# bioinfo-pf-curie/mpiBWA

Hardware: AMD Instinct MI355X
Metric: Mreads/s (whole node) 2x150 bp PE vs GRCh38-size reference; SAM bit-match (higher is better)
Workload: dtype int32

## Files before the change

mpibwa_amd/csrc/chain_kernel.hip:

```cpp
#include <hip/hip_runtime.h>
#include <hipcub/hipcub.hpp>
#include <cstdlib>
#include <mutex>
#include <utility>
#include <vector>
#include "hip_util.h"
#include "device.h"
#include "sortutil.h"

namespace mbw {

namespace {

typedef long long i64;

#define CK_MAXCH 9
#define CK_MAXCH_SMALL 4
#define CK_MAXSEEDS_SMALL 16
#define CK_MAXSEEDS 64
#define CK_MAXSEEDS_BIG 255
enum { F_POS_LO = 0, F_POS_HI, F_FIRST_Q, F_LAST_R_LO, F_LAST_R_HI, F_LAST_Q, F_LAST_LEN, F_RID, F_N, F_W, F_KEPT, F_FIRSTOV, F_NFIELDS };

template <int MAXCH>
struct StoreLds {
	uint32_t *tab;
	uint8_t *cid_;
	uint8_t *ord_;
	uint8_t *tmp_;
	int lane;
	__device__ __forceinline__ uint32_t &f(int field, int id) const { return tab[(field * MAXCH + id) * 64 + lane]; }
	__device__ __forceinline__ uint8_t &cid(int k) const { return cid_[k * 64 + lane]; }
	__device__ __forceinline__ uint8_t &ord(int k) const { return ord_[k * 64 + lane]; }
	__device__ __forceinline__ uint8_t &tmp(int k) const { return tmp_[k * 64 + lane]; }
};

template <int MAXCH> __device__ __forceinline__ i64 st_pos(const StoreLds<MAXCH> &L, int id) { return (i64)((unsigned long long)L.f(F_POS_HI, id) << 32 | L.f(F_POS_LO, id)); }
template <int MAXCH> __device__ __forceinline__ i64 st_last_r(const StoreLds<MAXCH> &L, int id) { return (i64)((unsigned long long)L.f(F_LAST_R_HI, id) << 32 | L.f(F_LAST_R_LO, id)); }

template <int MAXCH>
struct MapArray {
	int n = 0;
	__device__ __forceinline__ int lower(const StoreLds<MAXCH> &L, i64 pos) const
	{
		int f = 0;
		while (f < n && st_pos(L, L.ord(f)) < pos) ++f;
		const int li = (f < n && st_pos(L, L.ord(f)) == pos) ? f : f - 1;
		return li >= 0 ? (int)L.ord(li) : -1;
	}
	__device__ __forceinline__ bool put(const StoreLds<MAXCH> &L, int id, i64 pos)
	{
		if (n == MAXCH) return false;
		int f = 0;
		while (f < n && st_pos(L, L.ord(f)) < pos) ++f;
		const int li = (f < n && st_pos(L, L.ord(f)) == pos) ? f : f - 1;
		for (int t = n; t > li + 1; --t) L.ord(t) = L.ord(t - 1);
		L.ord(li + 1) = (uint8_t)id;
		++n;
		return true;
	}
};

__device__ __forceinline__ int ck_pos2rid(const i64 *__restrict__ ann_off, int n_seqs, i64 l_pac, i64 pos_f)
{
	if (pos_f >= l_pac) return -1;
	int left = 0, mid = 0, right = n_seqs;
	while (left < right) {
		mid = (left + right) >> 1;
		if (pos_f >= ann_off[mid]) {
			if (mid == n_seqs - 1 || pos_f < ann_off[mid + 1]) break;
			left = mid + 1;
		} else right = mid;
	}
	return mid;
}
__device__ __forceinline__ i64 ck_depos(i64 l_pac, i64 pos) { return pos >= l_pac ? (l_pac << 1) - 1 - pos : pos; }

template <int MAXCH>
__device__ __forceinline__ int chain_read(const StoreLds<MAXCH> &L, const ChainParams &P, int rd, int ns, int lq, i64 so, const int *__restrict__ l_rep,
                                          const unsigned long long *__restrict__ sa, const int32_t *__restrict__ qbl, const i64 *__restrict__ ann_off,
                                          const uint8_t *__restrict__ ann_alt, int n_seqs, const int *__restrict__ gap, DevChain *__restrict__ chains,
                                          DevSeed *__restrict__ seeds, unsigned int *__restrict__ srt)
{
	const i64 l_pac = P.l_pac;
	auto S_R = [&](int k) -> i64 { return (i64)sa[so + k]; };
	auto S_Q = [&](int k) -> int { return qbl[2 * (so + k)]; };
	auto S_L = [&](int k) -> int { return qbl[2 * (so + k) + 1]; };
	auto members = [&](int id, auto fn) {
		for (int k = 0; k < ns; ++k)
			if (L.cid(k) == id) fn(k);
	};

	MapArray<MAXCH> map;
	int n_ch = 0;
	i64 c_lo = 0, c_hi = -1;
	int c_rid = -1;
	for (int k = 0; k < ns; ++k) {
		const i64 rb = S_R(k);
		const int qb = S_Q(k), len = S_L(k);
		L.cid(k) = 255;
		int rid;
		if (rb >= c_lo && rb + len <= c_hi && len > 0) rid = c_rid;
		else {
			if (rb < l_pac && rb + len > l_pac) rid = -2;
			else {
				const int rid_b = ck_pos2rid(ann_off, n_seqs, l_pac, ck_depos(l_pac, rb));
				const int rid_e = len > 0 ? ck_pos2rid(ann_off, n_seqs, l_pac, ck_depos(l_pac, rb + len - 1)) : rid_b;
				rid = rid_b == rid_e ? rid_b : -1;
			}
			if (rid >= 0) {
				const i64 o = ann_off[rid], l = ann_off[rid + 1] - o;
				if (rb < l_pac) { c_lo = o; c_hi = o + l; }
				else { c_lo = (l_pac << 1) - o - l; c_hi = (l_pac << 1) - o; }
				c_rid = rid;
			}
		}
		if (rid < 0) continue;
		const int id0 = map.lower(L, rb);
		bool merged = false;
		if (id0 >= 0) {
			const int id = id0;
			const i64 first_r = st_pos(L, id), last_r = st_last_r(L, id);
			const int first_q = (int)L.f(F_FIRST_Q, id), last_q = (int)L.f(F_LAST_Q, id), last_len = (int)L.f(F_LAST_LEN, id);
			const int qend = last_q + last_len;
			const i64 rend = last_r + last_len;
			if ((int)L.f(F_RID, id) == rid) {
				if (qb >= first_q && qb + len <= qend && rb >= first_r && rb + len <= rend) merged = true;
				else if (!((last_r < l_pac || first_r < l_pac) && rb >= l_pac)) {
					const i64 x = qb - last_q, y = rb - last_r;
					if (y >= 0 && x - y <= P.w && y - x <= P.w && x - last_len < P.max_chain_gap && y - last_len < P.max_chain_gap) {
						L.f(F_LAST_R_LO, id) = (uint32_t)rb; L.f(F_LAST_R_HI, id) = (uint32_t)((unsigned long long)rb >> 32);
						L.f(F_LAST_Q, id) = (uint32_t)qb; L.f(F_LAST_LEN, id) = (uint32_t)len;
						L.f(F_N, id) += 1;
						L.cid(k) = (uint8_t)id;
						merged = true;
					}
				}
			}
		}
		if (merged) continue;
		const int id = n_ch;
		if (id >= MAXCH) return -1;
		L.f(F_POS_LO, id) = (uint32_t)rb; L.f(F_POS_HI, id) = (uint32_t)((unsigned long long)rb >> 32);
		L.f(F_FIRST_Q, id) = (uint32_t)qb;
		L.f(F_LAST_R_LO, id) = (uint32_t)rb; L.f(F_LAST_R_HI, id) = (uint32_t)((unsigned long long)rb >> 32);
		L.f(F_LAST_Q, id) = (uint32_t)qb; L.f(F_LAST_LEN, id) = (uint32_t)len;
		L.f(F_RID, id) = (uint32_t)rid; L.f(F_N, id) = 1;
		if (!map.put(L, id, rb)) return -1;
		L.cid(k) = (uint8_t)id;
		++n_ch;
	}

	int n = 0;
	for (int t = 0; t < n_ch; ++t) {
		const int id = L.ord(t);
		i64 end = 0;
		int w = 0, wq;
		members(id, [&](int k) {
			const int qb = S_Q(k), len = S_L(k);
			if (qb >= end) w += len;
			else if (qb + len > end) w += (int)(qb + len - end);
			end = end > qb + len ? end : qb + len;
		});
		wq = w; w = 0; end = 0;
		members(id, [&](int k) {
			const i64 rb = S_R(k);
			const int len = S_L(k);
			if (rb >= end) w += len;
			else if (rb + len > end) w += (int)(rb + len - end);
			end = end > rb + len ? end : rb + len;
		});
		w = w < wq ? w : wq;
		w = w < 1 << 30 ? w : (1 << 30) - 1;
		const uint32_t w29 = (uint32_t)w & 0x1fffffffu;
		L.f(F_W, id) = w29; L.f(F_KEPT, id) = 0; L.f(F_FIRSTOV, id) = 0xffffffffu;
		if ((int)w29 < P.min_chain_weight) continue;
		L.ord(n++) = (uint8_t)id;
	}
	if (n == 0) return 0;
	static_assert(MAXCH <= 16, "ks_small_introsort_at is ks_introsort for at most 16 elements");
	ks_small_introsort_at(n, [&](int k) -> uint8_t & { return L.ord(k); },
	                      [&](int a_id, int b_id) -> bool { return (int)L.f(F_W, a_id) > (int)L.f(F_W, b_id); });
	auto BEG = [&](int t) -> int { return (int)L.f(F_FIRST_Q, L.ord(t)); };
	auto END = [&](int t) -> int { const int id = L.ord(t); return (int)L.f(F_LAST_Q, id) + (int)L.f(F_LAST_LEN, id); };
	auto ALT = [&](int t) -> int { return ann_alt[L.f(F_RID, L.ord(t))]; };
	int n_kept = 0;
	L.f(F_KEPT, L.ord(0)) = 3;
	L.tmp(n_kept++) = 0;
	for (int i = 1; i < n; ++i) {
		bool large_ovlp = false;
		int kk;
		for (kk = 0; kk < n_kept; ++kk) {
			const int j = L.tmp(kk);
			const int b_max = BEG(j) > BEG(i) ? BEG(j) : BEG(i);
			const int e_min = END(j) < END(i) ? END(j) : END(i);
			if (e_min > b_max && (!ALT(j) || ALT(i))) {
				const int li_ = END(i) - BEG(i), lj_ = END(j) - BEG(j);
				const int min_l = li_ < lj_ ? li_ : lj_;
				if ((float)(e_min - b_max) >= (float)min_l * P.mask_level && min_l < P.max_chain_gap) {
					large_ovlp = true;
					if (L.f(F_FIRSTOV, L.ord(j)) == 0xffffffffu) L.f(F_FIRSTOV, L.ord(j)) = (uint32_t)i;
					const int wi = (int)L.f(F_W, L.ord(i)), wj = (int)L.f(F_W, L.ord(j));
					if ((float)wi < (float)wj * P.drop_ratio && wj - wi >= P.min_seed_len << 1) break;
				}
			}
		}
		if (kk == n_kept) {
			L.tmp(n_kept++) = (uint8_t)i;
			L.f(F_KEPT, L.ord(i)) = large_ovlp ? 2 : 3;
		}
	}
	for (int kk = 0; kk < n_kept; ++kk) {
		const uint32_t fo = L.f(F_FIRSTOV, L.ord(L.tmp(kk)));
		if (fo != 0xffffffffu) L.f(F_KEPT, L.ord(fo)) = 1;
	}
	{
		int i = 0, cnt = 0;
		for (; i < n; ++i) {
			const uint32_t kp = L.f(F_KEPT, L.ord(i));
			if (kp == 0 || kp == 3) continue;
			if (++cnt >= P.max_chain_extend) break;
		}
		for (; i < n; ++i)
			if (L.f(F_KEPT, L.ord(i)) < 3) L.f(F_KEPT, L.ord(i)) = 0;
	}

	const float frac_rep = (float)l_rep[rd] / (float)lq;
	int n_out = 0;
	i64 cursor = so;
	for (int t = 0; t < n; ++t) {
		const int id = L.ord(t);
		if (L.f(F_KEPT, id) == 0) continue;
		int cs = 0;
		members(id, [&](int k) { L.tmp(cs++) = (uint8_t)k; });
		for (int a = 1; a < cs; ++a) {
			const uint8_t v = L.tmp(a);
			const int lv = S_L(v);
			int b = a;
			while (b > 0 && S_L(L.tmp(b - 1)) > lv) { L.tmp(b) = L.tmp(b - 1); --b; }
			L.tmp(b) = v;
		}
		const int rid = (int)L.f(F_RID, id);
		const i64 first_r = st_pos(L, id);
		i64 lo = l_pac << 1, hi = 0;
		for (int a = 0; a < cs; ++a) {
			const int k = L.tmp(a);
			DevSeed ds;
			ds.rbeg = S_R(k); ds.qbeg = S_Q(k); ds.len = S_L(k);
			seeds[cursor + a] = ds;
			srt[cursor + a] = (unsigned int)a;
			const i64 b = ds.rbeg - (ds.qbeg + gap[ds.qbeg]);
			const int tail = lq - ds.qbeg - ds.len;
			const i64 e = ds.rbeg + ds.len + (tail + gap[tail]);
			lo = b < lo ? b : lo;
			hi = e > hi ? e : hi;
		}
		DevChain d;
		i64 fb = ann_off[rid], fe = ann_off[rid + 1];
		if (first_r >= l_pac) { const i64 tt = fb; fb = (l_pac << 1) - fe; fe = (l_pac << 1) - tt; }
		d.far_beg = fb; d.far_end = fe;
		d.seed_beg = (int)cursor; d.n_seeds = cs; d.rid = rid; d.frac_rep = frac_rep;
		d.rmax0 = lo > 0 ? lo : 0;
		d.rmax1 = hi < l_pac << 1 ? hi : l_pac << 1;
		if (d.rmax0 < l_pac && l_pac < d.rmax1) {
			if (first_r < l_pac) d.rmax1 = l_pac;
			else d.rmax0 = l_pac;
		}
		d.rmax0 = d.rmax0 > fb ? d.rmax0 : fb;
		d.rmax1 = d.rmax1 < fe ? d.rmax1 : fe;
		chains[so + n_out] = d;
		++n_out;
		cursor += cs;
	}
	return n_out;
}

template <int MAXS, int MAXCH, int LO>
__global__ void __launch_bounds__(64)
chain_kernel(ChainParams P, int n_reads, const int *__restrict__ lens, const int *__restrict__ n_seeds, const int *__restrict__ l_rep,
             const i64 *__restrict__ seed_off, const unsigned long long *__restrict__ sa, const int32_t *__restrict__ qbl,
             const i64 *__restrict__ ann_off, const uint8_t *__restrict__ ann_alt, int n_seqs, const int *__restrict__ tab, int tab_stride,
             DevChain *__restrict__ chains, DevSeed *__restrict__ seeds, unsigned int *__restrict__ srt, int *__restrict__ n_chains,
             const int *__restrict__ list, const unsigned int *__restrict__ list_n)
{
	extern __shared__ uint32_t lds_raw[];
	StoreLds<MAXCH> L;
	L.lane = threadIdx.x;
	L.tab = lds_raw;
	L.cid_ = (uint8_t *)(lds_raw + F_NFIELDS * MAXCH * 64);
	L.ord_ = L.cid_ + (MAXS + 1) * 64;
	L.tmp_ = L.ord_ + 16 * 64;
	int rd = blockIdx.x * 64 + threadIdx.x;
	if (list) { if (rd >= (int)*list_n) return; rd = list[rd]; }
	if (rd >= n_reads) return;
	const int ns = n_seeds[rd], lq = lens[rd];
	const int *gap = tab, *noflt = tab + 5 * tab_stride;
	if (LO >= 0) { if (n_chains[rd] != -1 || ns <= LO) return; }
	else if (ns == 0) { n_chains[rd] = 0; return; }
	if (ns > MAXS || !noflt[lq]) { n_chains[rd] = -1; return; }
	n_chains[rd] = chain_read(L, P, rd, ns, lq, seed_off[rd], l_rep, sa, qbl, ann_off, ann_alt, n_seqs, gap, chains, seeds, srt);
}

__global__ void __launch_bounds__(256)
chain_pick_kernel(int n_reads, const int *__restrict__ lens, const int *__restrict__ n_seeds, const int *__restrict__ n_chains,
                  const int *__restrict__ noflt, int lo, int hi, int cap, int *__restrict__ list, unsigned int *__restrict__ count)
{
	const int rd = blockIdx.x * 256 + threadIdx.x;
	const bool mine = rd < n_reads && n_chains[rd] == -1 && n_seeds[rd] > lo && n_seeds[rd] <= hi && noflt[lens[rd]] != 0;
	const unsigned long long m = __ballot(mine);
	if (!m) return;
	const int lane = threadIdx.x & 63, lead = __ffsll((long long)m) - 1;
	unsigned int base = 0;
	if (lane == lead) base = atomicAdd(count, (unsigned int)__popcll(m));
	base = __shfl(base, lead);
	const unsigned int at = base + (unsigned int)__popcll(m & ((1ull << lane) - 1));
	if (mine && at < (unsigned int)cap) list[at] = rd;
}

#define HV_NONE 0xFFFFu
__host__ __device__ constexpr size_t hv_lds_bytes(int cap) { return (size_t)(cap + 64) * 24; }
__host__ __device__ constexpr size_t hv_scratch_bytes(int cap) { return (size_t)cap * (4 + 7 * 2 + 8 + 4) + 512; }
struct HvStore {
	uint32_t *rid;
	uint16_t *head, *cid, *next, *ord;
	uint32_t *last_off;
	uint16_t *first_q, *last_q, *last_len, *tail, *nmem;
};
__device__ __forceinline__ bool hv_lt(uint32_t a, uint32_t b) { return (a >> 16) > (b >> 16); }
#define HV_FRAMES 32
__device__ __forceinline__ void hv_sort(uint32_t *a, int n)
{
	int fs[HV_FRAMES], ft[HV_FRAMES], fd[HV_FRAMES];
	ks_introsort_at(n, [a](int k) -> uint32_t & { return a[k]; }, KsFramesAt{fs, ft, fd}, hv_lt);
}
__device__ __forceinline__ void hv_sync()
{
	__builtin_amdgcn_fence(__ATOMIC_RELEASE, "wavefront");
	__builtin_amdgcn_wave_barrier();
	__builtin_amdgcn_fence(__ATOMIC_ACQUIRE, "wavefront");
}
__device__ __forceinline__ int hv_bcast(int v) { return __builtin_amdgcn_readfirstlane(v); }

template <int CAP>
__global__ void __launch_bounds__(64)
chain_heavy_kernel(ChainParams P, const int *__restrict__ list, const unsigned int *__restrict__ list_n, unsigned int *work, int list_cap,
                   const int *__restrict__ lens, const int *__restrict__ n_seeds, const int *__restrict__ l_rep, const i64 *__restrict__ seed_off,
                   const unsigned long long *__restrict__ sa, const int32_t *__restrict__ qbl, const i64 *__restrict__ ann_off,
                   const uint8_t *__restrict__ ann_alt, int n_seqs, const int *__restrict__ gap, uint8_t *__restrict__ scratch,
                   DevChain *__restrict__ chains, DevSeed *__restrict__ seeds, unsigned int *__restrict__ srt, int *__restrict__ n_chains)
{
	extern __shared__ uint8_t hv_lds[];
	const int lane = threadIdx.x;
	i64 *spos = (i64 *)hv_lds;
	uint16_t *sid = (uint16_t *)(hv_lds + (size_t)(CAP + 64) * 22);
	uint32_t *skey = (uint32_t *)hv_lds;
	uint16_t *cbeg = (uint16_t *)(skey + CAP);
	uint16_t *cend = cbeg + CAP, *kidx = cend + CAP, *kfirst = kidx + CAP;
	uint8_t *calt = (uint8_t *)(kfirst + CAP), *ckept = calt + CAP;
	uint8_t *sb = scratch + (size_t)blockIdx.x * hv_scratch_bytes(CAP);
	HvStore S;
	S.rid = (uint32_t *)sb;
	S.head = (uint16_t *)(S.rid + CAP); S.cid = S.head + CAP; S.next = S.cid + CAP; S.ord = S.next + CAP;
	S.last_off = (uint32_t *)(hv_lds + (size_t)(CAP + 64) * 8);
	S.first_q = (uint16_t *)(S.last_off + CAP); S.last_q = S.first_q + CAP; S.last_len = S.last_q + CAP; S.tail = S.last_len + CAP; S.nmem = S.tail + CAP;
	uint16_t *g_first_q = S.ord + CAP, *g_end_q = g_first_q + CAP, *g_nmem = g_end_q + CAP;
	i64 *g_clo = (i64 *)(sb + (((size_t)CAP * 18 + 15) & ~(size_t)15));
	int *g_rid = (int *)(g_clo + CAP);
	const i64 l_pac = P.l_pac;
	const int n_list = (int)(*list_n < (unsigned int)list_cap ? *list_n : (unsigned int)list_cap);
	for (;;) {
		int t = 0;
		if (lane == 0) t = (int)atomicAdd(work, 1u);
		t = hv_bcast(t);
		if (t >= n_list) break;
		const int rd = hv_bcast(list[t]);
		const int ns = hv_bcast(n_seeds[rd]), lq = hv_bcast(lens[rd]);
		const i64 so = seed_off[rd];
		auto S_R = [&](int k) -> i64 { return (i64)sa[so + k]; };
		auto S_Q = [&](int k) -> int { return qbl[2 * (so + k)]; };
		auto S_L = [&](int k) -> int { return qbl[2 * (so + k) + 1]; };
		if (ns > CAP) continue;
		int n_ch = 0, ok = 1;
		{
			for (int k = lane; k < ns; k += 64) {
				const i64 rb = S_R(k);
				const int len = S_L(k);
				int rid;
				if (rb < l_pac && rb + len > l_pac) rid = -2;
				else {
					const int rid_b = ck_pos2rid(ann_off, n_seqs, l_pac, ck_depos(l_pac, rb));
					const int rid_e = len > 0 ? ck_pos2rid(ann_off, n_seqs, l_pac, ck_depos(l_pac, rb + len - 1)) : rid_b;
					rid = rid_b == rid_e ? rid_b : -1;
				}
				i64 lo = -1;
				if (rid >= 0) lo = rb < l_pac ? ann_off[rid] : (l_pac << 1) - ann_off[rid + 1];
				g_rid[k] = rid; g_clo[k] = lo;
			}
			hv_sync();
			i64 nx_rb = S_R(0), nx_clo = g_clo[0];
			int nx_qb = S_Q(0), nx_len = S_L(0), nx_rid = g_rid[0];
			for (int k = 0; k < ns; ++k) {
				const i64 rb = nx_rb, c_lo = nx_clo;
				const int qb = nx_qb, len = nx_len, rid = nx_rid;
				if (k + 1 < ns) { nx_rb = S_R(k + 1); nx_qb = S_Q(k + 1); nx_len = S_L(k + 1); nx_rid = g_rid[k + 1]; nx_clo = g_clo[k + 1]; }
				if (rid < 0) { if (lane == 0) S.cid[k] = HV_NONE; continue; }
				int cnt;
				if (n_ch <= 64) cnt = __popcll(__ballot(lane < n_ch && spos[lane] <= rb));
				else {
					const int stride = (n_ch + 63) >> 6;
					const int at = lane * stride;
					const int blk = __popcll(__ballot(at < n_ch && spos[at] <= rb));
					if (blk == 0) cnt = 0;
					else {
						const int base = (blk - 1) * stride, e = base + lane;
						cnt = base + __popcll(__ballot(lane < stride && e < n_ch && spos[e] <= rb));
					}
				}
				bool merged = false;
				int id0 = -1;
				if (cnt > 0) {
					id0 = sid[cnt - 1];
					const i64 first_r = spos[cnt - 1];
					if (first_r >= c_lo) {
						const i64 last_r = first_r + (i64)S.last_off[id0];
						const int first_q = S.first_q[id0], last_q = S.last_q[id0], last_len = S.last_len[id0];
						const int qend = last_q + last_len;
						const i64 rend = last_r + last_len;
						if (qb >= first_q && qb + len <= qend && rb >= first_r && rb + len <= rend) { merged = true; if (lane == 0) S.cid[k] = HV_NONE; }
						else if (!((last_r < l_pac || first_r < l_pac) && rb >= l_pac)) {
							const i64 x = qb - last_q, y = rb - last_r;
							if (y >= 0 && x - y <= P.w && y - x <= P.w && x - last_len < P.max_chain_gap && y - last_len < P.max_chain_gap) {
								if (lane == 0) {
									S.last_off[id0] = (uint32_t)(rb - first_r); S.last_q[id0] = (uint16_t)qb; S.last_len[id0] = (uint16_t)len;
									S.nmem[id0] += 1;
									S.cid[k] = (uint16_t)id0;
									S.next[S.tail[id0]] = (uint16_t)k; S.next[k] = HV_NONE; S.tail[id0] = (uint16_t)k;
								}
								merged = true;
							}
						}
					}
				}
				if (!merged) {
					if (cnt > 0 && spos[cnt - 1] == rb) { ok = 0; break; }
					const int id = n_ch;
					for (int hi = n_ch; hi > cnt; hi -= 64) {
						const int e = hi - 1 - lane;
						i64 v = 0; uint16_t w = 0;
						if (e >= cnt) { v = spos[e]; w = sid[e]; }
						hv_sync();
						if (e >= cnt) { spos[e + 1] = v; sid[e + 1] = w; }
						hv_sync();
					}
					if (lane == 0) {
						spos[cnt] = rb; sid[cnt] = (uint16_t)id;
						S.last_off[id] = 0; S.rid[id] = (uint32_t)rid;
						S.first_q[id] = (uint16_t)qb; S.last_q[id] = (uint16_t)qb; S.last_len[id] = (uint16_t)len; S.nmem[id] = 1;
						S.head[id] = (uint16_t)k; S.tail[id] = (uint16_t)k; S.next[k] = HV_NONE;
						S.cid[k] = (uint16_t)id;
					}
					++n_ch;
				}
				hv_sync();
			}
			if (ok)
				for (int t0 = lane; t0 < n_ch; t0 += 64) S.ord[t0] = sid[t0];
		}
		ok = hv_bcast(ok); n_ch = hv_bcast(n_ch);
		hv_sync();
		if (!ok) { if (lane == 0) n_chains[rd] = -2; continue; }
		for (int id = lane; id < n_ch; id += 64) {
			g_first_q[id] = S.first_q[id]; g_end_q[id] = (uint16_t)(S.last_q[id] + S.last_len[id]); g_nmem[id] = S.nmem[id];
		}
		hv_sync();
		int n = 0;
		for (int t0 = 0; t0 < n_ch; t0 += 64) {
			const int tt = t0 + lane;
			int w = 0, id = 0;
			if (tt < n_ch) {
				id = S.ord[tt];
				i64 end = 0;
				int wq;
				for (int k = S.head[id]; k != HV_NONE; k = S.next[k]) {
					const int qb = S_Q(k), len = S_L(k);
					if (qb >= end) w += len;
					else if (qb + len > end) w += (int)(qb + len - end);
					end = end > qb + len ? end : qb + len;
				}
				wq = w; w = 0; end = 0;
				for (int k = S.head[id]; k != HV_NONE; k = S.next[k]) {
					const i64 rb = S_R(k);
					const int len = S_L(k);
					if (rb >= end) w += len;
					else if (rb + len > end) w += (int)(rb + len - end);
					end = end > rb + len ? end : rb + len;
				}
				w = w < wq ? w : wq;
			}
			const bool pass = tt < n_ch && w >= P.min_chain_weight && w < 65536;
			if (__ballot(tt < n_ch && w >= 65536)) ok = 0;
			const unsigned long long m = __ballot(pass);
			if (pass) skey[n + __popcll(m & ((1ull << lane) - 1))] = (uint32_t)w << 16 | (uint32_t)id;
			n += __popcll(m);
		}
		hv_sync();
		if (!ok) { if (lane == 0) n_chains[rd] = -2; continue; }
		if (n == 0) { if (lane == 0) n_chains[rd] = 0; continue; }
		static_assert((unsigned long long)CAP <= 16ull << HV_FRAMES, "ks_introsort_at: n <= 16 << FRAMES");
		if (lane == 0) hv_sort(skey, n);
		hv_sync();
		for (int t0 = 0; t0 < n; t0 += 64) {
			const int tt = t0 + lane;
			if (tt < n) {
				const int id = skey[tt] & 0xffff;
				cbeg[tt] = g_first_q[id];
				cend[tt] = g_end_q[id];
				calt[tt] = ann_alt[S.rid[id]];
				ckept[tt] = 0;
			}
		}
		if (lane == 0) { ckept[0] = 3; kidx[0] = 0; kfirst[0] = HV_NONE; }
		hv_sync();
		int nk = 1;
		for (int i = 1; i < n; ++i) {
			const int bi = cbeg[i], ei = cend[i], li = ei - bi, wi = (int)(skey[i] >> 16), alt_i = calt[i];
			bool large = false, broke = false;
			for (int k0 = 0; k0 < nk && !broke; k0 += 64) {
				const int kk = k0 + lane;
				bool sig = false, brk = false;
				if (kk < nk) {
					const int j = kidx[kk];
					const int bj = cbeg[j], ej = cend[j];
					const int b_max = bj > bi ? bj : bi, e_min = ej < ei ? ej : ei;
					if (e_min > b_max && (!calt[j] || alt_i)) {
						const int lj = ej - bj, min_l = li < lj ? li : lj;
						if ((float)(e_min - b_max) >= (float)min_l * P.mask_level && min_l < P.max_chain_gap) {
							sig = true;
							const int wj = (int)(skey[j] >> 16);
							brk = (float)wi < (float)wj * P.drop_ratio && wj - wi >= P.min_seed_len << 1;
						}
					}
				}
				unsigned long long sm = __ballot(sig);
				const unsigned long long bm = __ballot(brk);
				if (bm) {
					const int fb = __ffsll((long long)bm) - 1;
					sm &= fb == 63 ? ~0ull : ((2ull << fb) - 1);
					broke = true;
				}
				if (sm) {
					large = true;
					if ((sm >> lane) & 1) { if (kfirst[kk] == HV_NONE) kfirst[kk] = (uint16_t)i; }
				}
			}
			if (!broke) {
				if (lane == 0) { kidx[nk] = (uint16_t)i; kfirst[nk] = HV_NONE; ckept[i] = large ? 2 : 3; }
				++nk;
			}
			hv_sync();
		}
		for (int k0 = 0; k0 < nk; k0 += 64) {
			const int kk = k0 + lane;
			if (kk < nk && kfirst[kk] != HV_NONE) ckept[kfirst[kk]] = 1;
		}
		hv_sync();
		if (P.max_chain_extend < n) {
			if (lane == 0) {
				int i = 0, cnt = 0;
				for (; i < n; ++i) {
					if (ckept[i] == 0 || ckept[i] == 3) continue;
					if (++cnt >= P.max_chain_extend) break;
				}
				for (; i < n; ++i)
					if (ckept[i] < 3) ckept[i] = 0;
			}
			hv_sync();
		}
		const float frac_rep = (float)l_rep[rd] / (float)lq;
		int n_out = 0;
		i64 cursor = so;
		for (int t0 = 0; t0 < n; t0 += 64) {
			const int tt = t0 + lane;
			const bool kept = tt < n && ckept[tt] != 0;
			const int id = kept ? (int)(skey[tt] & 0xffff) : 0;
			const int cs = kept ? (int)g_nmem[id] : 0;
			int pre = cs;
			for (int o = 1; o < 64; o <<= 1) { const int v = __shfl_up(pre, o); if (lane >= o) pre += v; }
			const unsigned long long km = __ballot(kept);
			const i64 my_cur = cursor + (pre - cs);
			const int my_out = n_out + __popcll(km & ((1ull << lane) - 1));
			if (kept) {
				int a = 0;
				for (int k = S.head[id]; k != HV_NONE; k = S.next[k], ++a) {
					DevSeed ds;
					ds.rbeg = S_R(k); ds.qbeg = S_Q(k); ds.len = S_L(k);
					int b = a;
					while (b > 0 && seeds[my_cur + b - 1].len > ds.len) { seeds[my_cur + b] = seeds[my_cur + b - 1]; --b; }
					seeds[my_cur + b] = ds;
				}
				i64 lo = l_pac << 1, hi = 0;
				for (a = 0; a < cs; ++a) {
					const DevSeed ds = seeds[my_cur + a];
					srt[my_cur + a] = (unsigned int)a;
					const i64 b = ds.rbeg - (ds.qbeg + gap[ds.qbeg]);
					const int tail = lq - ds.qbeg - ds.len;
					const i64 e = ds.rbeg + ds.len + (tail + gap[tail]);
					lo = b < lo ? b : lo;
					hi = e > hi ? e : hi;
				}
				const int rid = (int)S.rid[id];
				const i64 first_r = S_R(S.head[id]);
				DevChain d;
				i64 fb = ann_off[rid], fe = ann_off[rid + 1];
				if (first_r >= l_pac) { const i64 x = fb; fb = (l_pac << 1) - fe; fe = (l_pac << 1) - x; }
				d.far_beg = fb; d.far_end = fe;
				d.seed_beg = (int)my_cur; d.n_seeds = cs; d.rid = rid; d.frac_rep = frac_rep;
				d.rmax0 = lo > 0 ? lo : 0;
				d.rmax1 = hi < l_pac << 1 ? hi : l_pac << 1;
				if (d.rmax0 < l_pac && l_pac < d.rmax1) {
					if (first_r < l_pac) d.rmax1 = l_pac;
					else d.rmax0 = l_pac;
				}
				d.rmax0 = d.rmax0 > fb ? d.rmax0 : fb;
				d.rmax1 = d.rmax1 < fe ? d.rmax1 : fe;
				chains[so + my_out] = d;
			}
			cursor += __shfl(pre, 63);
			n_out += __popcll(km);
		}
		if (lane == 0) n_chains[rd] = n_out;
		hv_sync();
	}
}

__global__ void reg_pack_kernel(int n_reads, const int *__restrict__ reg_beg, const int *__restrict__ n_regs, const int *__restrict__ reg_pos,
                                const DevReg *__restrict__ regs, DevReg *__restrict__ packed, C2aUnits U, const int *__restrict__ chain_beg,
                                const int *__restrict__ chain_cnt)
{
	const int r = blockIdx.x * blockDim.x + threadIdx.x;
	if (r >= n_reads) return;
	const int m = n_regs[r];
	DevReg *dst = packed + reg_pos[r];
	if (U.max_units > 0 && chain_cnt[r] > U.heavy_t) {
		int k = 0;
		for (int ci = chain_beg[r]; ci < chain_beg[r] + chain_cnt[r]; ++ci) {
			const DevReg *src = regs + U.c_rabs[ci];
			for (int j = 0; j < U.c_rcnt[ci]; ++j) dst[k++] = src[j];
		}
		return;
	}
	const DevReg *src = regs + reg_beg[r];
	for (int k = 0; k < m; ++k) dst[k] = src[k];
}

}

size_t reg_pack_tmp_bytes(int n_reads)
{
	size_t t = 0;
	HIP_OK(hipcub::DeviceScan::ExclusiveSum(nullptr, t, (const int *)nullptr, (int *)nullptr, n_reads + 1));
	return t + 256;
}

void launch_reg_pack(void *stream, int n_reads, const int *d_reg_beg, const int *d_nregs, int *d_reg_pos, const DevReg *d_regs, DevReg *d_packed,
                     void *d_tmp, size_t tmp_bytes, const C2aUnits *units, const int *d_chain_beg, const int *d_chain_cnt)
{
	C2aUnits U;
	if (units) U = *units;
	if (n_reads <= 0) return;
	HIP_OK(hipcub::DeviceScan::ExclusiveSum(d_tmp, tmp_bytes, d_nregs, d_reg_pos, n_reads + 1, (hipStream_t)stream));
	hipLaunchKernelGGL(reg_pack_kernel, dim3((n_reads + 255) / 256), dim3(256), 0, (hipStream_t)stream, n_reads, d_reg_beg, d_nregs, d_reg_pos, d_regs,
	                   d_packed, U, d_chain_beg, d_chain_cnt);
	HIP_OK(hipGetLastError());
}

static size_t chain_lds_bytes(int maxs, int maxch) { return (size_t)F_NFIELDS * maxch * 64 * 4 + (size_t)(2 * (maxs + 1) + 16) * 64; }

#define HV_WAVES_T 4096
#define HV_WAVES_S 1024
#define HV_WAVES_L 256
static size_t heavy_scratch_bytes() { return HV_WAVES_T * hv_scratch_bytes(256) + HV_WAVES_S * hv_scratch_bytes(1024) + HV_WAVES_L * hv_scratch_bytes(4096); }
size_t chain_scratch_bytes(int n_reads) { return (size_t)n_reads * 8 + 512 + (size_t)n_reads * 8 + 256 + heavy_scratch_bytes(); }

struct ChainSide { hipStream_t s[2]; hipEvent_t fork, join[2]; };
static ChainSide chain_side_streams(hipStream_t st)
{
	static std::mutex side_mu;
	static std::vector<std::pair<hipStream_t, ChainSide>> sides;
	std::lock_guard<std::mutex> lk(side_mu);
	for (auto &e : sides) if (e.first == st) return e.second;
	ChainSide sd;
	for (int k = 0; k < 2; ++k) { HIP_OK(hipStreamCreateWithFlags(&sd.s[k], hipStreamNonBlocking)); HIP_OK(hipEventCreateWithFlags(&sd.join[k], hipEventDisableTiming)); }
	HIP_OK(hipEventCreateWithFlags(&sd.fork, hipEventDisableTiming));
	sides.emplace_back(st, sd);
	return sd;
}

void launch_chain(void *stream, const ChainParams &P, int n_reads, const int *d_len, const int *d_nseeds, const int *d_lrep,
                  const int64_t *d_seed_off, const uint64_t *d_sa, const int32_t *d_qbl, const int64_t *d_ann_off, const uint8_t *d_ann_alt,
                  int n_seqs, const int *d_tab, int tab_stride, DevChain *d_chains, DevSeed *d_seeds, unsigned int *d_srt, int *d_nchains,
                  void *d_scratch)
{
	if (n_reads <= 0) return;
	const size_t lds_s = chain_lds_bytes(CK_MAXSEEDS_SMALL, CK_MAXCH_SMALL), lds = chain_lds_bytes(CK_MAXSEEDS, CK_MAXCH), lds_big = chain_lds_bytes(CK_MAXSEEDS_BIG, CK_MAXCH);
	static bool s_attr = false;
	if (!s_attr) {
		if (lds > 64 * 1024) HIP_OK(hipFuncSetAttribute((const void *)chain_kernel<CK_MAXSEEDS, CK_MAXCH, 0>, hipFuncAttributeMaxDynamicSharedMemorySize, (int)lds));
		if (lds_big > 64 * 1024) HIP_OK(hipFuncSetAttribute((const void *)chain_kernel<CK_MAXSEEDS_BIG, CK_MAXCH, CK_MAXSEEDS>, hipFuncAttributeMaxDynamicSharedMemorySize, (int)lds_big));
		s_attr = true;
	}
	hipStream_t st = (hipStream_t)stream;
	const dim3 grid((n_reads + 63) / 64), block(64);
#define CHAIN_ARGS P, n_reads, d_len, d_nseeds, d_lrep, (const i64 *)d_seed_off, (const unsigned long long *)d_sa, d_qbl, (const i64 *)d_ann_off, d_ann_alt, n_seqs, d_tab, \
	               tab_stride, d_chains, d_seeds, d_srt, d_nchains
#define LAUNCH_HEAVY(CAP, waves, s, list, n, work, scr)                                                                                                       \
	hipLaunchKernelGGL((chain_heavy_kernel<CAP>), dim3(waves), dim3(64), hv_lds_bytes(CAP), s, P, (const int *)(list), (const unsigned int *)(n), work,      \
	                   n_reads, d_len, d_nseeds, d_lrep, (const i64 *)d_seed_off, (const unsigned long long *)d_sa, d_qbl, (const i64 *)d_ann_off, d_ann_alt, \
	                   n_seqs, d_tab, scr, d_chains, d_seeds, d_srt, d_nchains)
	const int big = getenv("MPIBWA_CHAIN_BIG") ? atoi(getenv("MPIBWA_CHAIN_BIG")) : 2;
	int *list_a = (int *)d_scratch, *list_b = list_a + n_reads;
	unsigned int *count = (unsigned int *)(list_b + n_reads);
	int *list_h1 = (int *)((uint8_t *)count + 512), *list_h2 = list_h1 + n_reads;
	uint8_t *scr_t = (uint8_t *)(((uintptr_t)(list_h2 + n_reads) + 255) & ~(uintptr_t)255);
	uint8_t *scr_s = scr_t + HV_WAVES_T * hv_scratch_bytes(256), *scr_l = scr_s + HV_WAVES_S * hv_scratch_bytes(1024);
	HIP_OK(hipMemsetAsync(count, 0, 64, st));
	auto pick = [&](int lo, int hi, int *list, unsigned int *n) {
		hipLaunchKernelGGL(chain_pick_kernel, dim3((n_reads + 255) / 256), dim3(256), 0, st, n_reads, d_len, d_nseeds, (const int *)d_nchains, d_tab + 5 * tab_stride, lo, hi,
		                   n_reads, list, n);
	};
	hipLaunchKernelGGL((chain_kernel<CK_MAXSEEDS_SMALL, CK_MAXCH_SMALL, -1>), grid, block, lds_s, st, CHAIN_ARGS, (const int *)nullptr, (const unsigned int *)nullptr);
	pick(0, CK_MAXSEEDS, list_a, count + 1);
	hipLaunchKernelGGL((chain_kernel<CK_MAXSEEDS, CK_MAXCH, 0>), grid, block, lds, st, CHAIN_ARGS, (const int *)list_a, (const unsigned int *)(count + 1));
	if (big >= 1) {
		pick(CK_MAXSEEDS, CK_MAXSEEDS_BIG, list_b, count + 2);
		hipLaunchKernelGGL((chain_kernel<CK_MAXSEEDS_BIG, CK_MAXCH, CK_MAXSEEDS>), grid, block, lds_big, st, CHAIN_ARGS, (const int *)list_b, (const unsigned int *)(count + 2));
	}
	if (big >= 2) {
		int *list_t = list_a;
		pick(0, CK_MAXSEEDS_BIG, list_t, count);
		const bool heavy = !(getenv("MPIBWA_CHAIN_HEAVY") && atoi(getenv("MPIBWA_CHAIN_HEAVY")) == 0);
		ChainSide sd = {};
		if (heavy) {
			static bool s_attr2 = false;
			if (!s_attr2) {
				HIP_OK(hipFuncSetAttribute((const void *)chain_heavy_kernel<4096>, hipFuncAttributeMaxDynamicSharedMemorySize, (int)hv_lds_bytes(4096)));
				s_attr2 = true;
			}
			pick(CK_MAXSEEDS_BIG, 1024, list_h1, count + 4);
			pick(1024, 4096, list_h2, count + 6);
			sd = chain_side_streams(st);
			HIP_OK(hipEventRecord(sd.fork, st));
			for (int k = 0; k < 2; ++k) HIP_OK(hipStreamWaitEvent(sd.s[k], sd.fork, 0));
			LAUNCH_HEAVY(4096, HV_WAVES_L, sd.s[0], list_h2, count + 6, count + 7, scr_l);
			LAUNCH_HEAVY(1024, HV_WAVES_S, sd.s[1], list_h1, count + 4, count + 5, scr_s);
		}
		LAUNCH_HEAVY(256, HV_WAVES_T, st, list_t, count, count + 3, scr_t);
		if (heavy)
			for (int k = 0; k < 2; ++k) { HIP_OK(hipEventRecord(sd.join[k], sd.s[k])); HIP_OK(hipStreamWaitEvent(st, sd.join[k], 0)); }
	}
#undef LAUNCH_HEAVY
#undef CHAIN_ARGS
	HIP_OK(hipGetLastError());
}

}
```

Measured before the change: 6.830.

## Add mid-size heavy chain tier, resize wave grids, move sort frames to LDS

Splits the heavy chaining pass into four capacity tiers by adding a 2048-seed tier on a third side stream. It also resizes the persistent wave counts per tier from a CU count and LDS budget. The insertion shift in the chain walk now moves four 64-element strips per barrier pair, and the introsort frame stacks move from private arrays into LDS. An optional clock64 phase profiler, gated by an environment variable, is added. The changes trade more LDS per wave and an extra stream and list against fewer barriers, less private scratch and better load balance across tiers.

```diff
diff --git a/mpibwa_amd/csrc/chain_kernel.hip b/mpibwa_amd/csrc/chain_kernel.hip
--- a/mpibwa_amd/csrc/chain_kernel.hip
+++ b/mpibwa_amd/csrc/chain_kernel.hip
@@ -1,5 +1,6 @@
 #include <hip/hip_runtime.h>
 #include <hipcub/hipcub.hpp>
+#include <cstdio>
 #include <cstdlib>
 #include <mutex>
 #include <utility>
@@ -317,7 +318,9 @@
 }
 
 #define HV_NONE 0xFFFFu
-__host__ __device__ constexpr size_t hv_lds_bytes(int cap) { return (size_t)(cap + 64) * 24; }
+#define HV_FRAMES 32
+__host__ __device__ constexpr size_t hv_map_bytes(int cap) { return (size_t)(cap + 64) * 24; }
+__host__ __device__ constexpr size_t hv_lds_bytes(int cap) { return hv_map_bytes(cap) + 3 * HV_FRAMES * 4; }
 __host__ __device__ constexpr size_t hv_scratch_bytes(int cap) { return (size_t)cap * (4 + 7 * 2 + 8 + 4) + 512; }
 struct HvStore {
 	uint32_t *rid;
@@ -326,11 +329,10 @@
 	uint16_t *first_q, *last_q, *last_len, *tail, *nmem;
 };
 __device__ __forceinline__ bool hv_lt(uint32_t a, uint32_t b) { return (a >> 16) > (b >> 16); }
-#define HV_FRAMES 32
-__device__ __forceinline__ void hv_sort(uint32_t *a, int n)
-{
-	int fs[HV_FRAMES], ft[HV_FRAMES], fd[HV_FRAMES];
-	ks_introsort_at(n, [a](int k) -> uint32_t & { return a[k]; }, KsFramesAt{fs, ft, fd}, hv_lt);
+#define HV_SHIFT_K 4
+__device__ __forceinline__ void hv_sort(uint32_t *a, int n, int *frames)
+{
+	ks_introsort_at(n, [a](int k) -> uint32_t & { return a[k]; }, KsFramesAt{frames, frames + HV_FRAMES, frames + 2 * HV_FRAMES}, hv_lt);
 }
 __device__ __forceinline__ void hv_sync()
 {
@@ -339,6 +341,8 @@
 	__builtin_amdgcn_fence(__ATOMIC_ACQUIRE, "wavefront");
 }
 __device__ __forceinline__ int hv_bcast(int v) { return __builtin_amdgcn_readfirstlane(v); }
+
+enum { HV_P_PRE = 0, HV_P_WALK, HV_P_SHIFT, HV_P_WEIGHT, HV_P_SORT, HV_P_PAIR, HV_P_EMIT, HV_P_READS, HV_P_SEEDS, HV_P_CHAINS, HV_P_WORDS, HV_P_N };
 
 template <int CAP>
 __global__ void __launch_bounds__(64)
@@ -346,7 +350,7 @@
                    const int *__restrict__ lens, const int *__restrict__ n_seeds, const int *__restrict__ l_rep, const i64 *__restrict__ seed_off,
                    const unsigned long long *__restrict__ sa, const int32_t *__restrict__ qbl, const i64 *__restrict__ ann_off,
                    const uint8_t *__restrict__ ann_alt, int n_seqs, const int *__restrict__ gap, uint8_t *__restrict__ scratch,
-                   DevChain *__restrict__ chains, DevSeed *__restrict__ seeds, unsigned int *__restrict__ srt, int *__restrict__ n_chains)
+                   DevChain *__restrict__ chains, DevSeed *__restrict__ seeds, unsigned int *__restrict__ srt, int *__restrict__ n_chains, unsigned long long *prof)
 {
 	extern __shared__ uint8_t hv_lds[];
 	const int lane = threadIdx.x;
@@ -356,6 +360,10 @@
 	uint16_t *cbeg = (uint16_t *)(skey + CAP);
 	uint16_t *cend = cbeg + CAP, *kidx = cend + CAP, *kfirst = kidx + CAP;
 	uint8_t *calt = (uint8_t *)(kfirst + CAP), *ckept = calt + CAP;
+	int *frames = (int *)(hv_lds + hv_map_bytes(CAP));
+	static_assert((size_t)(CAP + 64) * 22 + (size_t)(CAP + 64) * 2 == hv_map_bytes(CAP) && (size_t)(CAP + 64) * 8 + (size_t)CAP * 14 <= (size_t)(CAP + 64) * 22 &&
+	              (size_t)CAP * 14 <= hv_map_bytes(CAP) && hv_map_bytes(CAP) % 4 == 0 && hv_lds_bytes(CAP) == hv_map_bytes(CAP) + 3 * HV_FRAMES * sizeof(int),
+	              "the frames lie behind the map and behind the filter's columns");
 	uint8_t *sb = scratch + (size_t)blockIdx.x * hv_scratch_bytes(CAP);
 	HvStore S;
 	S.rid = (uint32_t *)sb;
@@ -367,6 +375,11 @@
 	int *g_rid = (int *)(g_clo + CAP);
 	const i64 l_pac = P.l_pac;
 	const int n_list = (int)(*list_n < (unsigned int)list_cap ? *list_n : (unsigned int)list_cap);
+	i64 pf_last = 0, pf_shift = 0;
+	auto pf_add = [&](int what, i64 v) { if (lane == 0) atomicAdd(prof + what, (unsigned long long)v); };
+	auto pf_tick = [&](int phase) {
+		if (prof) { const i64 now = clock64(); pf_add(phase, now - pf_last); pf_last = now; }
+	};
 	for (;;) {
 		int t = 0;
 		if (lane == 0) t = (int)atomicAdd(work, 1u);
@@ -379,6 +392,7 @@
 		auto S_Q = [&](int k) -> int { return qbl[2 * (so + k)]; };
 		auto S_L = [&](int k) -> int { return qbl[2 * (so + k) + 1]; };
 		if (ns > CAP) continue;
+		if (prof) { pf_last = clock64(); pf_shift = 0; pf_add(HV_P_READS, 1); pf_add(HV_P_SEEDS, ns); }
 		int n_ch = 0, ok = 1;
 		{
 			for (int k = lane; k < ns; k += 64) {
@@ -396,6 +410,7 @@
 				g_rid[k] = rid; g_clo[k] = lo;
 			}
 			hv_sync();
+			pf_tick(HV_P_PRE);
 			i64 nx_rb = S_R(0), nx_clo = g_clo[0];
 			int nx_qb = S_Q(0), nx_len = S_L(0), nx_rid = g_rid[0];
 			for (int k = 0; k < ns; ++k) {
@@ -443,14 +458,25 @@
 				if (!merged) {
 					if (cnt > 0 && spos[cnt - 1] == rb) { ok = 0; break; }
 					const int id = n_ch;
-					for (int hi = n_ch; hi > cnt; hi -= 64) {
-						const int e = hi - 1 - lane;
-						i64 v = 0; uint16_t w = 0;
-						if (e >= cnt) { v = spos[e]; w = sid[e]; }
+					i64 pf_t0 = 0;
+					if (prof) pf_t0 = clock64();
+					for (int hi = n_ch; hi > cnt; hi -= 64 * HV_SHIFT_K) {
+						i64 v[HV_SHIFT_K]; uint16_t w[HV_SHIFT_K];
+#pragma unroll
+						for (int j = 0; j < HV_SHIFT_K; ++j) {
+							const int e = hi - 1 - (j * 64 + lane);
+							v[j] = 0; w[j] = 0;
+							if (e >= cnt) { v[j] = spos[e]; w[j] = sid[e]; }
+						}
 						hv_sync();
-						if (e >= cnt) { spos[e + 1] = v; sid[e + 1] = w; }
+#pragma unroll
+						for (int j = 0; j < HV_SHIFT_K; ++j) {
+							const int e = hi - 1 - (j * 64 + lane);
+							if (e >= cnt) { spos[e + 1] = v[j]; sid[e + 1] = w[j]; }
+						}
 						hv_sync();
 					}
+					if (prof) pf_shift += clock64() - pf_t0;
 					if (lane == 0) {
 						spos[cnt] = rb; sid[cnt] = (uint16_t)id;
 						S.last_off[id] = 0; S.rid[id] = (uint32_t)rid;
@@ -467,6 +493,7 @@
 		}
 		ok = hv_bcast(ok); n_ch = hv_bcast(n_ch);
 		hv_sync();
+		if (prof) { pf_tick(HV_P_WALK); pf_add(HV_P_SHIFT, pf_shift); pf_add(HV_P_CHAINS, n_ch); }
 		if (!ok) { if (lane == 0) n_chains[rd] = -2; continue; }
 		for (int id = lane; id < n_ch; id += 64) {
 			g_first_q[id] = S.first_q[id]; g_end_q[id] = (uint16_t)(S.last_q[id] + S.last_len[id]); g_nmem[id] = S.nmem[id];
@@ -503,11 +530,13 @@
 			n += __popcll(m);
 		}
 		hv_sync();
+		if (prof) { pf_tick(HV_P_WEIGHT); pf_add(HV_P_WORDS, n); }
 		if (!ok) { if (lane == 0) n_chains[rd] = -2; continue; }
 		if (n == 0) { if (lane == 0) n_chains[rd] = 0; continue; }
 		static_assert((unsigned long long)CAP <= 16ull << HV_FRAMES, "ks_introsort_at: n <= 16 << FRAMES");
-		if (lane == 0) hv_sort(skey, n);
+		if (lane == 0) hv_sort(skey, n, frames);
 		hv_sync();
+		pf_tick(HV_P_SORT);
 		for (int t0 = 0; t0 < n; t0 += 64) {
 			const int tt = t0 + lane;
 			if (tt < n) {
@@ -575,6 +604,7 @@
 			}
 			hv_sync();
 		}
+		pf_tick(HV_P_PAIR);
 		const float frac_rep = (float)l_rep[rd] / (float)lq;
 		int n_out = 0;
 		i64 cursor = so;
@@ -629,6 +659,7 @@
 		}
 		if (lane == 0) n_chains[rd] = n_out;
 		hv_sync();
+		pf_tick(HV_P_EMIT);
 	}
 }
 
@@ -675,13 +706,21 @@
 
 static size_t chain_lds_bytes(int maxs, int maxch) { return (size_t)F_NFIELDS * maxch * 64 * 4 + (size_t)(2 * (maxs + 1) + 16) * 64; }
 
-#define HV_WAVES_T 4096
-#define HV_WAVES_S 1024
-#define HV_WAVES_L 256
-static size_t heavy_scratch_bytes() { return HV_WAVES_T * hv_scratch_bytes(256) + HV_WAVES_S * hv_scratch_bytes(1024) + HV_WAVES_L * hv_scratch_bytes(4096); }
-size_t chain_scratch_bytes(int n_reads) { return (size_t)n_reads * 8 + 512 + (size_t)n_reads * 8 + 256 + heavy_scratch_bytes(); }
-
-struct ChainSide { hipStream_t s[2]; hipEvent_t fork, join[2]; };
+#define HV_CUS 256
+#define HV_WAVES_T (20 * HV_CUS)
+#define HV_WAVES_S (6 * HV_CUS)
+#define HV_WAVES_M (3 * HV_CUS)
+#define HV_WAVES_L (1 * HV_CUS)
+static_assert(HV_WAVES_T / HV_CUS * hv_lds_bytes(256) <= 160 * 1024 && HV_WAVES_S / HV_CUS * hv_lds_bytes(1024) <= 160 * 1024 &&
+              HV_WAVES_M / HV_CUS * hv_lds_bytes(2048) <= 160 * 1024 && hv_lds_bytes(4096) <= 160 * 1024, "resident waves per CU by LDS");
+static size_t heavy_scratch_bytes()
+{
+	return HV_WAVES_T * hv_scratch_bytes(256) + HV_WAVES_S * hv_scratch_bytes(1024) + HV_WAVES_M * hv_scratch_bytes(2048) + HV_WAVES_L * hv_scratch_bytes(4096);
+}
+size_t chain_scratch_bytes(int n_reads) { return (size_t)n_reads * 8 + 512 + (size_t)n_reads * 12 + 256 + heavy_scratch_bytes(); }
+
+#define HV_SIDES 3
+struct ChainSide { hipStream_t s[HV_SIDES]; hipEvent_t fork, join[HV_SIDES]; };
 static ChainSide chain_side_streams(hipStream_t st)
 {
 	static std::mutex side_mu;
@@ -689,7 +728,7 @@
 	std::lock_guard<std::mutex> lk(side_mu);
 	for (auto &e : sides) if (e.first == st) return e.second;
 	ChainSide sd;
-	for (int k = 0; k < 2; ++k) { HIP_OK(hipStreamCreateWithFlags(&sd.s[k], hipStreamNonBlocking)); HIP_OK(hipEventCreateWithFlags(&sd.join[k], hipEventDisableTiming)); }
+	for (int k = 0; k < HV_SIDES; ++k) { HIP_OK(hipStreamCreateWithFlags(&sd.s[k], hipStreamNonBlocking)); HIP_OK(hipEventCreateWithFlags(&sd.join[k], hipEventDisableTiming)); }
 	HIP_OK(hipEventCreateWithFlags(&sd.fork, hipEventDisableTiming));
 	sides.emplace_back(st, sd);
 	return sd;
@@ -712,17 +751,24 @@
 	const dim3 grid((n_reads + 63) / 64), block(64);
 #define CHAIN_ARGS P, n_reads, d_len, d_nseeds, d_lrep, (const i64 *)d_seed_off, (const unsigned long long *)d_sa, d_qbl, (const i64 *)d_ann_off, d_ann_alt, n_seqs, d_tab, \
 	               tab_stride, d_chains, d_seeds, d_srt, d_nchains
-#define LAUNCH_HEAVY(CAP, waves, s, list, n, work, scr)                                                                                                       \
+#define LAUNCH_HEAVY(CAP, waves, s, list, n, work, scr, pf)                                                                                                     \
 	hipLaunchKernelGGL((chain_heavy_kernel<CAP>), dim3(waves), dim3(64), hv_lds_bytes(CAP), s, P, (const int *)(list), (const unsigned int *)(n), work,      \
 	                   n_reads, d_len, d_nseeds, d_lrep, (const i64 *)d_seed_off, (const unsigned long long *)d_sa, d_qbl, (const i64 *)d_ann_off, d_ann_alt, \
-	                   n_seqs, d_tab, scr, d_chains, d_seeds, d_srt, d_nchains)
+	                   n_seqs, d_tab, scr, d_chains, d_seeds, d_srt, d_nchains, pf)
 	const int big = getenv("MPIBWA_CHAIN_BIG") ? atoi(getenv("MPIBWA_CHAIN_BIG")) : 2;
 	int *list_a = (int *)d_scratch, *list_b = list_a + n_reads;
 	unsigned int *count = (unsigned int *)(list_b + n_reads);
-	int *list_h1 = (int *)((uint8_t *)count + 512), *list_h2 = list_h1 + n_reads;
-	uint8_t *scr_t = (uint8_t *)(((uintptr_t)(list_h2 + n_reads) + 255) & ~(uintptr_t)255);
-	uint8_t *scr_s = scr_t + HV_WAVES_T * hv_scratch_bytes(256), *scr_l = scr_s + HV_WAVES_S * hv_scratch_bytes(1024);
-	HIP_OK(hipMemsetAsync(count, 0, 64, st));
+	int *list_h1 = (int *)((uint8_t *)count + 512), *list_h2 = list_h1 + n_reads, *list_h3 = list_h2 + n_reads;
+	uint8_t *scr_t = (uint8_t *)(((uintptr_t)(list_h3 + n_reads) + 255) & ~(uintptr_t)255);
+	uint8_t *scr_s = scr_t + HV_WAVES_T * hv_scratch_bytes(256), *scr_m = scr_s + HV_WAVES_S * hv_scratch_bytes(1024);
+	uint8_t *scr_l = scr_m + HV_WAVES_M * hv_scratch_bytes(2048);
+	const bool s_prof = getenv("MPIBWA_CHAIN_PROF") && atoi(getenv("MPIBWA_CHAIN_PROF")) != 0;
+	static const int prof_caps[] = {256, 1024, 2048, 4096};
+	constexpr int N_PROF = (int)(sizeof(prof_caps) / sizeof(prof_caps[0]));
+	static_assert(128 + N_PROF * HV_P_N * 8 <= 512, "the phase table lies in the 512 bytes of the counters");
+	unsigned long long *prof = s_prof ? (unsigned long long *)(count + 32) : nullptr;
+	auto prof_of = [&](int k) { return prof ? prof + k * HV_P_N : nullptr; };
+	HIP_OK(hipMemsetAsync(count, 0, s_prof ? 512 : 64, st));
 	auto pick = [&](int lo, int hi, int *list, unsigned int *n) {
 		hipLaunchKernelGGL(chain_pick_kernel, dim3((n_reads + 255) / 256), dim3(256), 0, st, n_reads, d_len, d_nseeds, (const int *)d_nchains, d_tab + 5 * tab_stride, lo, hi,
 		                   n_reads, list, n);
@@ -746,20 +792,37 @@
 				s_attr2 = true;
 			}
 			pick(CK_MAXSEEDS_BIG, 1024, list_h1, count + 4);
-			pick(1024, 4096, list_h2, count + 6);
+			pick(1024, 2048, list_h3, count + 8);
+			pick(2048, 4096, list_h2, count + 6);
 			sd = chain_side_streams(st);
 			HIP_OK(hipEventRecord(sd.fork, st));
-			for (int k = 0; k < 2; ++k) HIP_OK(hipStreamWaitEvent(sd.s[k], sd.fork, 0));
-			LAUNCH_HEAVY(4096, HV_WAVES_L, sd.s[0], list_h2, count + 6, count + 7, scr_l);
-			LAUNCH_HEAVY(1024, HV_WAVES_S, sd.s[1], list_h1, count + 4, count + 5, scr_s);
-		}
-		LAUNCH_HEAVY(256, HV_WAVES_T, st, list_t, count, count + 3, scr_t);
+			for (int k = 0; k < HV_SIDES; ++k) HIP_OK(hipStreamWaitEvent(sd.s[k], sd.fork, 0));
+			LAUNCH_HEAVY(4096, HV_WAVES_L, sd.s[0], list_h2, count + 6, count + 7, scr_l, prof_of(3));
+			LAUNCH_HEAVY(2048, HV_WAVES_M, sd.s[2], list_h3, count + 8, count + 9, scr_m, prof_of(2));
+			LAUNCH_HEAVY(1024, HV_WAVES_S, sd.s[1], list_h1, count + 4, count + 5, scr_s, prof_of(1));
+		}
+		LAUNCH_HEAVY(256, HV_WAVES_T, st, list_t, count, count + 3, scr_t, prof_of(0));
 		if (heavy)
-			for (int k = 0; k < 2; ++k) { HIP_OK(hipEventRecord(sd.join[k], sd.s[k])); HIP_OK(hipStreamWaitEvent(st, sd.join[k], 0)); }
+			for (int k = 0; k < HV_SIDES; ++k) { HIP_OK(hipEventRecord(sd.join[k], sd.s[k])); HIP_OK(hipStreamWaitEvent(st, sd.join[k], 0)); }
 	}
 #undef LAUNCH_HEAVY
 #undef CHAIN_ARGS
 	HIP_OK(hipGetLastError());
-}
-
-}
+	if (prof && big >= 2) {
+		unsigned long long h[N_PROF * HV_P_N];
+		HIP_OK(hipStreamSynchronize(st));
+		HIP_OK(hipMemcpy(h, prof, sizeof(h), hipMemcpyDeviceToHost));
+		for (int k = 0; k < N_PROF; ++k) {
+			const unsigned long long *c = h + k * HV_P_N;
+			double all = 0;
+			for (int ph = HV_P_PRE; ph <= HV_P_EMIT; ++ph) if (ph != HV_P_SHIFT) all += (double)c[ph];
+			const double pc = all > 0 ? 100.0 / all : 0.0;
+			fprintf(stderr, "[chain] heavy<%d>: %llu reads, %llu seeds, %llu chains, %llu sort words; %.0f ticks of lane 0: contigs %.1f %%, walk %.1f %% "
+			        "(of it shifts %.1f %%), weight %.1f %%, sort %.1f %%, pairwise %.1f %%, emission %.1f %%\n", prof_caps[k], c[HV_P_READS], c[HV_P_SEEDS],
+			        c[HV_P_CHAINS], c[HV_P_WORDS], all, pc * c[HV_P_PRE], pc * c[HV_P_WALK], pc * c[HV_P_SHIFT], pc * c[HV_P_WEIGHT], pc * c[HV_P_SORT],
+			        pc * c[HV_P_PAIR], pc * c[HV_P_EMIT]);
+		}
+	}
+}
+
+}
```

After: 7.321 (median of 6 runs). 1.07x the previous value.
